# Alanlee0323/ISWM

Measured on AMD Instinct MI355X. Metric: training images/sec (513x513) DeepLabV3+-ResNet101, higher is better.
Workload: dtype f32; 1 GPU; deeplabv3plus_resnet101 output_stride=16, 513x513 synthetic tiles, 16 images/GPU (BASELINE.json configs[2]: global batch 128 over 8 GPUs), weighted CE [1,3], SGD-nesterov + cosine LR; fp32 tensors, conv products via six bf16 MFMAs on an exact 3-way operand split (bf16x6, fp32-level error); conv_math=bf16x6, global_batch=16, parallelism=dp1

## Files before the change

include/iswm_hip.h:

```cpp
#ifndef ISWM_HIP_H
#define ISWM_HIP_H

#include <stddef.h>
#include <stdint.h>

#ifdef __cplusplus
extern "C" {
#endif

typedef void* iswm_stream_t;

const char* iswm_last_error(void);
int iswm_version(void);

typedef struct {
    int N, H, W, Cin;
    int Ho, Wo, Cout;
    int KH, KW, stride, pad, dil;
    int ldx;
    int ldy;
} iswm_conv_desc;

int iswm_set_conv_math(int mode);
int iswm_get_conv_math(void);
// ... 25 lines not shown
int iswm_conv2d_dgrad_packed(const iswm_conv_desc* d, const float* dy, const void* wpk, float* dx, int accumulate,
                             iswm_stream_t stream);
int iswm_split_planes(const float* x, int64_t M, int C, int ldx, void* planes, int ldp, int64_t plane_stride,
                      iswm_stream_t stream);
int iswm_join_planes(const void* planes, int ldp, int64_t plane_stride, int64_t M, int C, float* x, int ldx,
                     iswm_stream_t stream);
int iswm_bn_apply_pl(const float* y, int64_t M, int C, int ldy, const float* scale, const float* shift, const float* mean,
                     const void* residual, int ldr, int64_t res_ps, int relu, void* out, int ldo, int64_t out_ps,
                     iswm_stream_t stream);
int iswm_bn_backward_pl(const float* dout, int ldd, const void* out, int ldo, int64_t out_ps, const float* y, int ldy,
                        int64_t M, int C, const float* mean, const float* invstd, const float* gamma,
                        const float* mask_scale, const float* mask_shift, int relu, int training, float* dgamma,
                        float* dbeta, void* dy, int lddy, int64_t dy_ps, float* dres, int lddres, void* workspace,
                        size_t workspace_bytes, iswm_stream_t stream);
int iswm_maxpool3x3s2_fwd_pl(const float* x, int N, int H, int W, int C, void* y, int64_t y_ps, uint8_t* idx, int Ho,
                             int Wo, iswm_stream_t stream);
int iswm_gap_fwd_pl(const void* x, int64_t x_ps, int N, int HW, int C, int ldx, float* y, iswm_stream_t stream);
int iswm_bcast_fwd_pl(const float* v, int N, int HW, int C, void* y, int ldy, int64_t y_ps, iswm_stream_t stream);
int iswm_bilinear_fwd_pl(const float* x, int N, int Hi, int Wi, int C, int ldx, void* y, int64_t y_ps, int Ho, int Wo,
                         int ldy, iswm_stream_t stream);
size_t iswm_conv2d_pl2_weight_bytes(const iswm_conv_desc* d, int kind);
int iswm_conv2d_pl2_pack_weights(const iswm_conv_desc* d, int kind, const float* w, void* packed, iswm_stream_t stream);
int iswm_conv2d_pl2_tile_rows(const iswm_conv_desc* d, int kind);
int iswm_conv2d_fwd_pl2(const iswm_conv_desc* d, const void* xp, int64_t plane_stride, const void* wpk,
                        const float* bias, float* y, float* stat_partials, iswm_stream_t stream);
int iswm_conv2d_dgrad_pl2(const iswm_conv_desc* d, const void* dyp, int64_t plane_stride, const void* wpk,
                          float* dx, int accumulate, iswm_stream_t stream);
int iswm_conv2d_dgrad_pl2_stat_tiles(const iswm_conv_desc* d);
int iswm_conv2d_dgrad_pl2_bn(const iswm_conv_desc* d, const void* dyp, int64_t plane_stride, const void* wpk, float* dx,
                             int accumulate, const float* y, int ldy, const float* mean, const float* invstd,
                             const float* mask_scale, const float* mask_shift, int relu, const void* mask_hi,
                             int ld_mask, double* partials, int tiles, iswm_stream_t stream);
int iswm_bn_backward_stats_pl(const float* dout, int ldd, const void* out, int ldo, int64_t out_ps, const float* y, int ldy,
                              int64_t M, int C, const float* mean, const float* invstd, const float* gamma,
                              const float* mask_scale, const float* mask_shift, int relu, int training, float* dgamma,
                              float* dbeta, void* dy, int lddy, int64_t dy_ps, float* dres, int lddres,
                              const double* partials, int tiles, void* workspace, size_t workspace_bytes,
                              iswm_stream_t stream);
size_t iswm_aspp_plan_bytes(const iswm_conv_desc* d, int nbranch, const int* ksize, const int* dil, int kind);
int iswm_aspp_plan(const iswm_conv_desc* d, int nbranch, const int* ksize, const int* dil, int kind, void* host_plan,
                   int grid_hint);
int iswm_aspp_fwd(const iswm_conv_desc* d, int nbranch, const int* ksize, const int* dil, const void* plan_dev, const void* xp,
                  int64_t x_ps, const void* const* wpk, float* const* y, float* const* stats, iswm_stream_t stream);
int iswm_aspp_bwd(const iswm_conv_desc* d, int nbranch, const int* ksize, const int* dil, const void* plan_dev, const void* dyp,
                  int64_t dy_ps, int ld_dy, const void* const* wpk, float* dx, int accumulate, const void* xp, int64_t x_ps,
                  float* const* dw, float* workspace, size_t workspace_bytes, iswm_stream_t stream);
// ... 198 lines not shown
```

iswm_amd/_lib.py:

```python
import ctypes
import os
from ctypes import POINTER, Structure, c_char_p, c_double, c_float, c_int, c_int64, c_size_t, c_uint64, c_void_p

HERE = os.path.dirname(os.path.abspath(__file__))
LIB_PATH = os.path.join(HERE, "libiswm_hip.so")


class ConvDesc(Structure):
    _fields_ = [(n, c_int) for n in ("N", "H", "W", "Cin", "Ho", "Wo", "Cout", "KH", "KW", "stride", "pad",
                                     "dil", "ldx", "ldy")]


class QConvDesc(Structure):
    _fields_ = [(n, c_int) for n in ("N", "H", "W", "Cin", "Ho", "Wo", "Cout", "KH", "KW", "stride", "pad",
                                     "dil", "ldx", "ldy", "ldr", "relu", "lo", "out_f32", "cstore")]


P = c_void_p
_SIGS = {
    "iswm_last_error": (c_char_p, []),
    "iswm_version": (c_int, []),
    "iswm_set_conv_math": (c_int, [c_int]),
    "iswm_get_conv_math": (c_int, []),
    "iswm_conv2d_kernel_name": (c_int, [POINTER(ConvDesc), c_int, c_char_p, c_int]),
# ... 4 lines not shown
    "iswm_transpose_weights": (c_int, [POINTER(ConvDesc), P, P, P]),
    "iswm_conv2d_dgrad_wants_wt": (c_int, [POINTER(ConvDesc)]),
    "iswm_conv2d_dgrad_wt": (c_int, [POINTER(ConvDesc), P, P, P, c_int, P]),
    "iswm_conv2d_packed_weight_bytes": (c_size_t, [POINTER(ConvDesc), c_int]),
    "iswm_conv2d_pack_weights": (c_int, [POINTER(ConvDesc), c_int, P, P, P]),
    "iswm_packed_weight_bytes": (c_size_t, [c_int, c_int, c_int, c_int]),
    "iswm_pack_job_blocks": (c_int, [c_int, c_int, c_int, c_int]),
    "iswm_pack_weights_batch": (c_int, [P, c_int, c_int, P]),
    "iswm_conv2d_fwd_packed_stat_layout": (c_int, [POINTER(ConvDesc), POINTER(c_int), POINTER(c_int)]),
    "iswm_conv2d_fwd_packed": (c_int, [POINTER(ConvDesc), P, P, P, P, P, P]),
    "iswm_conv2d_dgrad_packed": (c_int, [POINTER(ConvDesc), P, P, P, c_int, P]),
    "iswm_split_planes": (c_int, [P, c_int64, c_int, c_int, P, c_int, c_int64, P]),
    "iswm_join_planes": (c_int, [P, c_int, c_int64, c_int64, c_int, P, c_int, P]),
    "iswm_bn_apply_pl": (c_int, [P, c_int64, c_int, c_int, P, P, P, P, c_int, c_int64, c_int, P, c_int, c_int64, P]),
    "iswm_bn_backward_pl": (c_int, [P, c_int, P, c_int, c_int64, P, c_int, c_int64, c_int, P, P, P, P, P, c_int, c_int, P, P, P,
                                    c_int, c_int64, P, c_int, P, c_size_t, P]),
    "iswm_maxpool3x3s2_fwd_pl": (c_int, [P, c_int, c_int, c_int, c_int, P, c_int64, P, c_int, c_int, P]),
    "iswm_gap_fwd_pl": (c_int, [P, c_int64, c_int, c_int, c_int, c_int, P, P]),
    "iswm_bcast_fwd_pl": (c_int, [P, c_int, c_int, c_int, P, c_int, c_int64, P]),
    "iswm_bilinear_fwd_pl": (c_int, [P, c_int, c_int, c_int, c_int, c_int, P, c_int64, c_int, c_int, c_int, P]),
    "iswm_conv2d_pl2_weight_bytes": (c_size_t, [POINTER(ConvDesc), c_int]),
    "iswm_conv2d_pl2_pack_weights": (c_int, [POINTER(ConvDesc), c_int, P, P, P]),
    "iswm_conv2d_pl2_tile_rows": (c_int, [POINTER(ConvDesc), c_int]),
    "iswm_conv2d_fwd_pl2": (c_int, [POINTER(ConvDesc), P, c_int64, P, P, P, P, P]),
    "iswm_conv2d_dgrad_pl2": (c_int, [POINTER(ConvDesc), P, c_int64, P, P, c_int, P]),
    "iswm_conv2d_dgrad_pl2_stat_tiles": (c_int, [POINTER(ConvDesc)]),
    "iswm_conv2d_dgrad_pl2_bn": (c_int, [POINTER(ConvDesc), P, c_int64, P, P, c_int, P, c_int, P, P, P, P, c_int, P, c_int, P,
                                         c_int, P]),
    "iswm_bn_backward_stats_pl": (c_int, [P, c_int, P, c_int, c_int64, P, c_int, c_int64, c_int, P, P, P, P, P, c_int, c_int, P, P,
                                          P, c_int, c_int64, P, c_int, P, c_int, P, c_size_t, P]),
    "iswm_aspp_plan_bytes": (c_size_t, [POINTER(ConvDesc), c_int, POINTER(c_int), POINTER(c_int), c_int]),
    "iswm_aspp_plan": (c_int, [POINTER(ConvDesc), c_int, POINTER(c_int), POINTER(c_int), c_int, P, c_int]),
    "iswm_aspp_fwd": (c_int, [POINTER(ConvDesc), c_int, POINTER(c_int), POINTER(c_int), P, P, c_int64, POINTER(c_void_p),
                              POINTER(c_void_p), POINTER(c_void_p), P]),
    "iswm_aspp_bwd": (c_int, [POINTER(ConvDesc), c_int, POINTER(c_int), POINTER(c_int), P, P, c_int64, c_int, POINTER(c_void_p), P,
                              c_int, P, c_int64, POINTER(c_void_p), P, c_size_t, P]),
    "iswm_conv2d_wgrad_planes_ok": (c_int, [POINTER(ConvDesc)]),
    "iswm_conv2d_wgrad_planes_workspace": (c_size_t, [POINTER(ConvDesc)]),
    "iswm_conv2d_wgrad_planes": (c_int, [POINTER(ConvDesc), P, c_int64, P, c_int64, P, P, c_size_t, P]),
    "iswm_conv2d_wgrad_workspace": (c_size_t, [POINTER(ConvDesc)]),
    "iswm_dwconv2d_fwd": (c_int, [POINTER(ConvDesc), P, P, c_int, P, P, P]),
    "iswm_dwconv2d_dgrad": (c_int, [POINTER(ConvDesc), P, P, c_int, P, c_int, P]),
    "iswm_dwconv2d_wgrad_workspace": (c_size_t, [POINTER(ConvDesc)]),
    "iswm_dwconv2d_wgrad": (c_int, [POINTER(ConvDesc), P, P, c_int, P, P, c_size_t, P]),
    "iswm_dwconv3x3_stat_tile_rows": (c_int, [POINTER(ConvDesc)]),
    "iswm_dwconv3x3_stat_tiles": (c_int, [POINTER(ConvDesc)]),
# ... 114 lines not shown
```

iswm_amd/csrc/conv_api.hip:

```cpp
#include <stdlib.h>
#include <string.h>

#include <atomic>

#include "conv_common.h"

using namespace iswm;

static std::atomic<int> g_conv_math{-1};
static int conv_math() {
    int m = g_conv_math.load();
    if (m < 0) {
        const char* e = getenv("ISWM_CONV_MATH");
        const int env = (e && (!strcmp(e, "f32") || !strcmp(e, "0"))) ? 0
                        : (e && (!strcmp(e, "bf16") || !strcmp(e, "2"))) ? 2 : 1;
        int unset = -1;
        g_conv_math.compare_exchange_strong(unset, env);
        m = g_conv_math.load();
    }
    return m;
}
extern "C" int iswm_set_conv_math(int mode) {
    ISWM_REQUIRE(mode >= 0 && mode <= 2, "set_conv_math: mode must be 0 (f32), 1 (bf16x6) or 2 (bf16)");
    g_conv_math = mode;
// ... 200 lines not shown
    return route_name(plan_route(d, kind == 1 && dgrad_wants_wt(d, math) ? E_DGRAD_WT : entry[kind], math), buf, buflen);
}

extern "C" int iswm_conv2d_stat_tile_rows(const iswm_conv_desc* d) {
    return d ? plan_route(d, E_FWD, conv_math()).tile_rows : 0;
}

extern "C" int iswm_conv2d_stat_tiles(const iswm_conv_desc* d) {
    return d ? plan_route(d, E_FWD, conv_math()).tiles : 0;
}

extern "C" int iswm_conv2d_fwd_packed_stat_layout(const iswm_conv_desc* d, int* tiles, int* tile_rows) {
    ISWM_REQUIRE(d && tiles && tile_rows, "fwd_packed_stat_layout: null pointer");
    const ConvRoute r = plan_route(d, E_FWD_PACKED, conv_math());
    *tiles = r.tiles;
    *tile_rows = r.tile_rows;
    return 0;
}

extern "C" int iswm_conv2d_pl2_tile_rows(const iswm_conv_desc* d, int kind) {
    return d ? plan_route(d, kind ? E_DGRAD_PL2 : E_FWD_PL2, conv_math()).tile_rows : 0;
}

extern "C" int iswm_conv2d_dgrad_pl2_stat_tiles(const iswm_conv_desc* d) {
    return (d && d->Cin > 0) ? plan_route(d, E_DGRAD_PL2, conv_math()).stat_tiles : 0;
}

extern "C" size_t iswm_conv2d_wgrad_workspace(const iswm_conv_desc* d) {
    return d ? plan_wgrad(d, conv_math()).workspace : 0;
}

extern "C" int iswm_conv2d_fwd(const iswm_conv_desc* d, const float* x, const float* w, const float* bias,
                               float* y, float* stat_partials, iswm_stream_t stream) {
    if (int e = validate(d)) return e;
    ISWM_REQUIRE(x && w && y, "conv_fwd: null pointer");
    ISWM_REQUIRE(aligned16(x) && aligned16(w) && aligned16(y), "conv_fwd: pointers must be 16-byte aligned");
    ConvArgs a = base_args(d);
    a.x = x; a.w = w; a.bias = bias; a.y = y; a.stats = stat_partials;
    hipStream_t s = (hipStream_t)stream;
    const ConvRoute r = plan_route(d, E_FWD, conv_math());
    switch (r.family) {
    case F_STEM:
        ISWM_REQUIRE(launch_stem_fwd(a, s), "conv_fwd: the stem kernel does not cover this geometry");
        return check_launch("stem_fwd");
    case F_X6:
        ISWM_REQUIRE(launch_conv_fwd_x6(a, s, r.bm, r.bn), "conv_fwd: no bf16x6 kernel for tile %d x %d", r.bm, r.bn);
// ... 243 lines not shown
```

iswm_amd/csrc/conv_common.h:

```cpp
#pragma once
#include <stdlib.h>
#include "common.h"
#include "planes.h"

namespace iswm {

typedef float f32x16 __attribute__((ext_vector_type(16)));

struct BnFuse {
    const float* y;
    const float* mean;
    const float* invstd;
    const float* mscale;
    const float* mshift;
    double* part;
    int ldy, relu;
    const unsigned short* mask;
    int ldm;
};

struct ConvArgs {
    const float* x;
    const float* w;
    const float* bias;
// ... 96 lines not shown
    for (int i = 0; i < 8; ++i) {
        float x = 0.f;
        if (col < NC) x = DGRAD ? w[((size_t)(g0 + i) * T + tap) * Cin + col] : w[((size_t)col * T + tap) * Cin + g0 + i];
        v[i] = x;
    }
    uint4* o = packed + (size_t)f * (64 * NP) + lane;
    if constexpr (NP == 1) {
        const uint2 r0 = round_bf16x4(make_float4(v[0], v[1], v[2], v[3])), r1 = round_bf16x4(make_float4(v[4], v[5], v[6], v[7]));
        o[0] = make_uint4(r0.x, r0.y, r1.x, r1.y);
    } else {
        uint2 h0, m0, l0, h1, m1, l1;
        split3(make_float4(v[0], v[1], v[2], v[3]), h0, m0, l0);
        split3(make_float4(v[4], v[5], v[6], v[7]), h1, m1, l1);
        o[0] = make_uint4(h0.x, h0.y, h1.x, h1.y);
        o[64] = make_uint4(m0.x, m0.y, m1.x, m1.y);
        o[128] = make_uint4(l0.x, l0.y, l1.x, l1.y);
    }
}

int pack_job_blocks_pl2(int Cout, int T, int Cin, bool dgrad);
void conv_pl2_plan(int64_t M, int cols, int K, bool wide_ok, int* rbw, int* wide, int* wm);
bool launch_conv_pl2w(ConvArgs a, hipStream_t s, bool dgrad, int planes, int rbw);
bool launch_conv_pl2(ConvArgs a, hipStream_t s, bool dgrad, int planes, int rbw, int wm);
size_t packed_weight_bytes_pl2(int Cout, int T, int Cin, bool dgrad, int planes);
void launch_pack_weights_pl2(const float* w, void* packed, int Cout, int T, int Cin, bool dgrad, int planes, hipStream_t s);

struct PatchArgs {
    const float* x;
    const uint4* wpk;
    const float* bias;
    float* y;
    float* stats;
    int N, RH, RW;
    int GH, GW;
    int GC, NC;
    int KH, KW, dil;
    int orgh, orgw;
    int flip;
    int PH, PW, HH, HW;
    int TPY, TPX;
    int ldg, ldo;
    int MT, NT;
    int accumulate;
};
bool conv_patch_plan(int RH, int RW, int KH, int KW, int dil, int* PH, int* PW);
void launch_conv_x6_patch(PatchArgs a, bool dgrad, int planes, hipStream_t s);
// ... 28 lines not shown
```

iswm_amd/csrc/conv_mfma_pl2.hip:

```cpp
#include <stdlib.h>

#include "conv_pl2_stage.h"

namespace iswm {

constexpr int PL2_RBWMAX = 10;
constexpr double PL2W_EFF = 0.85;

template <int RBW, int WM, int NP, bool DGRAD>
__global__ __launch_bounds__(512, 2) void k_conv_pl2(const ConvArgs a) {
    const int GC = DGRAD ? a.Cout : a.Cin;
    const int NC = DGRAD ? a.Cin : a.Cout;
    constexpr int WN = 8 / WM, BN = 16 * WN;
    using S = Pl2Stage<16 * RBW * WM, NP>;
    constexpr int BM = S::BM, RG = S::RG, NRG = S::NRG, PLANE = S::PLANE, STAGE = S::STAGE;
    constexpr int XTRA = (DGRAD ? BM * 4 : 0) + (WM > 1 ? 4 * 128 * 4 : 0);
    __shared__ __attribute__((aligned(1024))) unsigned char smem[2 * STAGE + XTRA];
    int* rowpix = reinterpret_cast<int*>(smem + 2 * STAGE);
    float* red = reinterpret_cast<float*>(smem + 2 * STAGE + (DGRAD ? BM * 4 : 0));
    const unsigned lds_base = (unsigned)(uintptr_t)(lds_vptr)smem;

    const int t = threadIdx.x, lane = t & 63;
    const int wave = __builtin_amdgcn_readfirstlane(t >> 6);
    const int wm = wave / WN, wn = wave - wm * WN;
    const bool par = DGRAD && a.stride == 2 && a.psplit == 0;
    const int RH = DGRAD ? a.H : a.Ho, RW = DGRAD ? a.W : a.Wo;
    const int GH = DGRAD ? a.Ho : a.H, GW = DGRAD ? a.Wo : a.W;
    const int taps = a.KH * a.KW;
    const int nCC = GC >> 6;
    const int K32 = a.Ktot >> 5;
    const int ntiles = a.MT * a.NT;
    const unsigned char* xb = reinterpret_cast<const unsigned char*>(a.x);
    const int gs = pl2_dma_group(lane, wave);
    const unsigned char* zrow = reinterpret_cast<const unsigned char*>(g_zero_row_pl2) + gs * 16;

    int i_tile = xcd_remap(blockIdx.x, gridDim.x);
    int i_m0 = 0, i_n0 = 0;
    int ihb[NRG], iwb[NRG], pb[NRG];
    const uint4* wpk = nullptr;
    auto par_mt = [&](int sq) __attribute__((always_inline)) -> int {
        const int qn = a.MT >> 2, rem = a.MT & 3;
        int k = 0;
#pragma unroll
        for (int j = 0; j < 4; ++j) {
            k = (a.porder >> (2 * j)) & 3;
            const int sz = qn + (k < rem ? 1 : 0);
            if (sq < sz || j == 3) break;
            sq -= sz;
        }
        return k * qn + (k < rem ? k : rem) + sq;
    };
    auto load_tile = [&](int tile) __attribute__((always_inline)) {
        int mt = tile / a.NT;
        const int nt = tile - mt * a.NT;
        if (par) mt = par_mt(mt);
        i_m0 = mt * BM;
        i_n0 = nt * BN;
#pragma unroll
        for (int i = 0; i < NRG; ++i) {
            const int m = i_m0 + 8 * (wave + 8 * i) + (lane >> 3);
            if (wave + 8 * i < RG && m < a.M) {
                int n, rh, rw;
                x6_row_pixel(m, a.N, RH, RW, par, n, rh, rw);
                ihb[i] = DGRAD ? rh + a.pad : rh * a.stride - a.pad;
                iwb[i] = DGRAD ? rw + a.pad : rw * a.stride - a.pad;
                pb[i] = n * GH * GW;
            } else {
                ihb[i] = PL2_NO_ROW;
                iwb[i] = 0;
                pb[i] = 0;
            }
        }
        wpk = reinterpret_cast<const uint4*>(a.w) + (size_t)((i_n0 >> 4) + wn) * K32 * (64 * NP) + lane;
    };
    const unsigned char* aptr[NRG];
    int astep[NRG];
    long long pst[NRG];
    auto setup_tap = [&](int tap) __attribute__((always_inline)) -> bool {
        const int kh = tap / a.KW, kw = tap - kh * a.KW;
        const int dh = kh * a.dil, dw = kw * a.dil;
        int any = 0;
#pragma unroll
        for (int i = 0; i < NRG; ++i) {
            int gh, gw;
            bool ok;
            if (DGRAD) {
                int th = ihb[i] - dh, tw = iwb[i] - dw;
                gh = th;
                gw = tw;
                ok = th >= 0 && tw >= 0;
                if (a.stride != 1) {
                    gh = th / a.stride;
                    gw = tw / a.stride;
                    ok = ok && (gh * a.stride == th) && (gw * a.stride == tw);
                }
                ok = ok && gh < GH && gw < GW;
            } else {
                gh = ihb[i] + dh;
                gw = iwb[i] + dw;
                ok = (unsigned)gh < (unsigned)GH && (unsigned)gw < (unsigned)GW;
            }
// ... 53 lines not shown
            asrc[i] = more ? aptr[i] : zrow;
            apl[i] = more ? pst[i] : 0;
        }
        auto slot = [&](int sidx) __attribute__((always_inline)) {
            if (sidx < NB_SLOTS) {
                bn.v[sidx / NP][sidx % NP] = wn_[sidx * 64];
            } else if (sidx < NSLOTS) {
                const int i = (sidx - NB_SLOTS) / NP, pp = (sidx - NB_SLOTS) % NP;
                if (8 * i + 8 <= RG || wave + 8 * i < RG)
                    glds16b(asrc[i] + pp * apl[i], lds_base + (st ^ 1) * STAGE + pp * PLANE + (wave + 8 * i) * 1024);
                if (pp == NP - 1) aptr[i] += astep[i];
            }
        };
        Pl2AFrag<NP> f[3];
        pl2_aload<S, RBW>(f[0], smem, st, fbase, 0);
        pl2_aload<S, RBW>(f[1], smem, st, fbase, 1);
#pragma unroll
        for (int idx = 0; idx < 2 * RBW; ++idx) {
            if (idx + 2 < 2 * RBW) pl2_aload<S, RBW>(f[(idx + 2) % 3], smem, st, fbase, idx + 2);
            __builtin_amdgcn_sched_barrier(0);
            pl2_mul(acc[idx % RBW], b.v[idx / RBW], f[idx % 3]);
#pragma unroll
            for (int q = 0; q < PER; ++q) slot(idx * PER + q);
            __builtin_amdgcn_sched_barrier(0);
        }
    };

    const int lq = lane >> 4, lp = lane & 15;
    auto epilogue = [&](int tile, int m0, int n0, bool zero) __attribute__((always_inline)) {
        int mt = tile / a.NT;
        if (par) mt = par_mt(mt);
        const int col = n0 + 16 * wn + 4 * lq;
        const bool cok = col < NC;
        const bool bnf = DGRAD && a.bnf.part != nullptr;
        const bool mk = bnf && a.bnf.relu == 3;
        if (DGRAD && a.accumulate && zero && !bnf) return;
        float4 bv = make_float4(0.f, 0.f, 0.f, 0.f);
        if (!DGRAD && a.bias != nullptr && cok) bv = *reinterpret_cast<const float4*>(a.bias + col);
        if (DGRAD && par) {
            __syncthreads();
            if (t < BM) {
                const int m = m0 + t;
                int n = 0, rh = 0, rw = 0;
                if (m < a.M) x6_row_pixel(m, a.N, RH, RW, true, n, rh, rw);
                rowpix[DGRAD ? t : 0] = (n * RH + rh) * RW + rw;
            }
// ... 172 lines not shown
            for (int i = 0; i < RBW; ++i) acc[i] = f32x4{0.f, 0.f, 0.f, 0.f};
        }
    };

    int c_tile = i_tile, c_m0, c_n0;
    load_tile(i_tile);
    c_m0 = i_m0;
    c_n0 = i_n0;
    auto next_tile = [&]() __attribute__((always_inline)) -> bool {
        i_tile += gridDim.x;
        if (i_tile >= ntiles) return false;
        load_tile(i_tile);
        tap = -1;
        cc = nCC - 1;
        return true;
    };
    auto next_tile_stage = [&]() __attribute__((always_inline)) -> bool {
        for (;;) {
            if (!next_tile()) return false;
            if (next_in_tile()) return true;
            epilogue(i_tile, i_m0, i_n0, true);
        }
    };
    {
        BFrag bc, bn;
        bool have = next_in_tile();
        if (!have) {
            epilogue(i_tile, i_m0, i_n0, true);
            have = next_tile_stage();
            c_tile = i_tile; c_m0 = i_m0; c_n0 = i_n0;
        }
        if (have) {
            bload(bc, tap * (GC >> 5) + 2 * cc);
            issueA(0);
        }
        int st = 0;
        while (have) {
            __builtin_amdgcn_s_waitcnt(0x0F70);
            __builtin_amdgcn_s_barrier();
            asm volatile("" ::: "memory");
            bool more = next_in_tile();
            const bool last = !more;
            if (last) more = next_tile_stage();
            compute(st, bc, more, bn, more ? tap * (GC >> 5) + 2 * cc : 0);
            if (last) {
                epilogue(c_tile, c_m0, c_n0, false);
                c_tile = i_tile; c_m0 = i_m0; c_n0 = i_n0;
// ... 20 lines not shown
            best = rbw;
        }
    }
    return best;
}

void conv_pl2_plan(int64_t M, int cols, int K, bool wide_ok, int* rbw_out, int* wide_out, int* wm_out) {
    *wm_out = cols <= 64 ? 2 : 1;
    *rbw_out = conv_pl2_pick_rbw(M, cols, *wm_out);
    *wide_out = 0;
    if (!wide_ok || cols < 256 || K < 256) return;
    const int64_t NT = (cols + 127) / 128, NTW = (cols + 255) / 256;
    const int64_t MT0 = (M + *rbw_out * 16 - 1) / (*rbw_out * 16);
    double best = (double)((MT0 * NT + 255) / 256) * (*rbw_out * 16 + 24.0);
    for (int rbw = 8; rbw <= PL2_RBWMAX; ++rbw) {
        const int64_t MT = (M + rbw * 16 - 1) / (rbw * 16);
        const double c = (double)((MT * NTW + 255) / 256) * (rbw * 16 + 24.0) * 2.0 * PL2W_EFF;
        if (c < best - 1e-9) {
            best = c;
            *rbw_out = rbw;
            *wide_out = 1;
        }
    }
}

bool launch_conv_pl2(ConvArgs a, hipStream_t s, bool dgrad, int planes, int rbw, int wm) {
    a.psplit = 0;
    {
        int wgt[4], ord[4] = {0, 1, 2, 3};
        for (int k = 0; k < 4; ++k) {
            int ch = 0, cw = 0;
            for (int kh = 0; kh < a.KH; ++kh) ch += (((k >> 1) + a.pad - kh * a.dil) & 1) == 0;
            for (int kw = 0; kw < a.KW; ++kw) cw += (((k & 1) + a.pad - kw * a.dil) & 1) == 0;
            wgt[k] = ch * cw;
        }
        for (int i = 0; i < 4; ++i)
            for (int j = i + 1; j < 4; ++j)
                if (wgt[ord[j]] > wgt[ord[i]]) { const int t = ord[i]; ord[i] = ord[j]; ord[j] = t; }
        a.porder = ord[0] | (ord[1] << 2) | (ord[2] << 4) | (ord[3] << 6);
    }
    const int nc = dgrad ? a.Cin : a.Cout;
    const bool narrow = wm == 2;
    a.MT = (a.M + rbw * 16 - 1) / (rbw * 16);
    a.NT = narrow ? 1 : (nc + 127) / 128;
    const int tiles = a.MT * a.NT, ncu = device_cus();
    dim3 grid(tiles < ncu ? tiles : ncu), blk(512);
    if (planes != 1 && planes != 3) return false;
#define PL2_LAUNCH(R, W)                                                                       \
    do {                                                                                       \
        if (planes == 1) {                                                                     \
            if (dgrad) hipLaunchKernelGGL((k_conv_pl2<R, W, 1, true>), grid, blk, 0, s, a);     \
            else hipLaunchKernelGGL((k_conv_pl2<R, W, 1, false>), grid, blk, 0, s, a);          \
        } else {                                                                               \
            if (dgrad) hipLaunchKernelGGL((k_conv_pl2<R, W, 3, true>), grid, blk, 0, s, a);     \
            else hipLaunchKernelGGL((k_conv_pl2<R, W, 3, false>), grid, blk, 0, s, a);          \
        }                                                                                      \
    } while (0)
    if (narrow) {
        if (rbw == 8) PL2_LAUNCH(4, 2);
        else if (rbw == 10) PL2_LAUNCH(5, 2);
        else return false;
    } else {
        if (rbw == 8) PL2_LAUNCH(8, 1);
        else if (rbw == 9) PL2_LAUNCH(9, 1);
        else if (rbw == 10) PL2_LAUNCH(10, 1);
        else return false;
    }
#undef PL2_LAUNCH
    return true;
}

template <bool DGRAD, int NP>
__global__ __launch_bounds__(256) void k_pack_weights_pl2(const float* __restrict__ w, uint4* __restrict__ packed, int Cout,
                                                          int T, int Cin, int K32, int total) {
    const int idx = blockIdx.x * 256 + threadIdx.x;
    if (idx >= total) return;
    pack_weights_pl2_body<DGRAD, NP>(w, packed, Cout, T, Cin, K32, idx);
}

int pack_job_blocks_pl2(int Cout, int T, int Cin, bool dgrad) {
    const int NC = dgrad ? Cin : Cout, GC = dgrad ? Cout : Cin;
// ... 27 lines not shown
```

iswm_amd/csrc/conv_mfma_pl2w.hip:

```cpp
#include <stdlib.h>

#include "conv_pl2_stage.h"

namespace iswm {

template <int RBW, int NP, bool DGRAD>
__global__ __launch_bounds__(512, 2) void k_conv_pl2w(const ConvArgs a) {
    const int GC = DGRAD ? a.Cout : a.Cin;
    const int NC = DGRAD ? a.Cin : a.Cout;
    using S = Pl2Stage<16 * RBW, NP>;
    constexpr int BM = S::BM, RG = S::RG, NRG = S::NRG, PLANE = S::PLANE, STAGE = S::STAGE;
    __shared__ __attribute__((aligned(1024))) unsigned char smem[2 * STAGE];
    const unsigned lds_base = (unsigned)(uintptr_t)(lds_vptr)smem;

    const int t = threadIdx.x, lane = t & 63;
    const int wave = __builtin_amdgcn_readfirstlane(t >> 6);
    const int RH = DGRAD ? a.H : a.Ho, RW = DGRAD ? a.W : a.Wo;
    const int GH = DGRAD ? a.Ho : a.H, GW = DGRAD ? a.Wo : a.W;
    const int taps = a.KH * a.KW;
    const int nCC = GC >> 6;
    const int K32 = a.Ktot >> 5;
    const int ntiles = a.MT * a.NT;
    const int cbs = ((NC + 127) >> 7) << 3;
    const unsigned char* xb = reinterpret_cast<const unsigned char*>(a.x);
    const int gs = pl2_dma_group(lane, wave);
    const unsigned char* zrow = reinterpret_cast<const unsigned char*>(g_zero_row_pl2) + gs * 16;

    int i_tile = xcd_remap(blockIdx.x, gridDim.x);
    int i_m0 = 0, i_n0 = 0;
    int ihb[NRG], iwb[NRG], pb[NRG];
    const uint4* wpk[2] = {nullptr, nullptr};
    auto load_tile = [&](int tile) __attribute__((always_inline)) {
        const int mt = tile / a.NT;
        const int nt = tile - mt * a.NT;
        i_m0 = mt * BM;
        i_n0 = nt * 256;
#pragma unroll
        for (int i = 0; i < NRG; ++i) {
            const int m = i_m0 + 8 * (wave + 8 * i) + (lane >> 3);
            if (wave + 8 * i < RG && m < a.M) {
                int n, rh, rw;
                x6_row_pixel(m, a.N, RH, RW, false, n, rh, rw);
                ihb[i] = DGRAD ? rh + a.pad : rh * a.stride - a.pad;
                iwb[i] = DGRAD ? rw + a.pad : rw * a.stride - a.pad;
                pb[i] = n * GH * GW;
            } else {
                ihb[i] = PL2_NO_ROW;
                iwb[i] = 0;
                pb[i] = 0;
            }
        }
#pragma unroll
        for (int cb = 0; cb < 2; ++cb) {
            const int cbi = min((i_n0 >> 4) + 2 * wave + cb, cbs - 1);
            wpk[cb] = reinterpret_cast<const uint4*>(a.w) + (size_t)cbi * K32 * (64 * NP) + lane;
        }
    };
    const unsigned char* aptr[NRG];
    int astep[NRG];
    long long pst[NRG];
    auto setup_tap = [&](int tap) __attribute__((always_inline)) -> bool {
        const int kh = tap / a.KW, kw = tap - kh * a.KW;
        const int dh = kh * a.dil, dw = kw * a.dil;
        int any = 0;
#pragma unroll
        for (int i = 0; i < NRG; ++i) {
            int gh, gw;
            bool ok;
            if (DGRAD) {
                gh = ihb[i] - dh;
                gw = iwb[i] - dw;
                ok = gh >= 0 && gw >= 0 && gh < GH && gw < GW;
            } else {
                gh = ihb[i] + dh;
                gw = iwb[i] + dw;
                ok = (unsigned)gh < (unsigned)GH && (unsigned)gw < (unsigned)GW;
            }
            aptr[i] = ok ? xb + ((size_t)(pb[i] + gh * GW + gw) * a.ldx) * 2 + gs * 16 : zrow;
            astep[i] = ok ? 128 : 0;
            pst[i] = ok ? a.xps : 0;
            any |= ok;
        }
        if (a.pad < 4) return true;
        return __syncthreads_or(any) != 0;
// ... 75 lines not shown
                const int cb = s / NP, pl = s - cb * NP;
                if (half == 0) B[cb][1][pl] = (cb ? wc1 : wc0)[(NP + pl) * 64];
                else B[cb][0][pl] = (cb ? wn1 : wn0)[pl * 64];
            } else {
                const int j = s - NB;
                if (half == 0) { if (j < NA0) dma(j); }
                else { if (j < NA1) dma(NA0 + j); }
            }
        };
        Pl2AFrag<NP> f[3];
        aload(f[0], 0);
        aload(f[1], 1);
#pragma unroll
        for (int idx = 0; idx < 2 * RBW; ++idx) {
            if (idx + 2 < 2 * RBW) aload(f[(idx + 2) % 3], idx + 2);
            __builtin_amdgcn_sched_barrier(0);
            mul(f[idx % 3], idx);
            const int half = idx / RBW, rb = idx - half * RBW;
            slot(half, 2 * rb);
            slot(half, 2 * rb + 1);
            __builtin_amdgcn_sched_barrier(0);
        }
        static_assert(2 * RBW >= NB + NA1, "load slots do not fit the row blocks of a k half");
    };

    const int lq = lane >> 4, lp = lane & 15;
    auto epilogue = [&](int tile, int m0, int n0, bool zero) __attribute__((always_inline)) {
        const int mt = tile / a.NT;
        const bool bnf = DGRAD && a.bnf.part != nullptr;
        const bool mk = bnf && a.bnf.relu == 3;
        if (DGRAD && a.accumulate && zero && !bnf) return;
#pragma unroll
        for (int cb = 0; cb < 2; ++cb) {
            const int col = n0 + 32 * wave + 16 * cb + 4 * lq;
            const bool cok = col < NC;
            float4 bv = make_float4(0.f, 0.f, 0.f, 0.f);
            if (!DGRAD && a.bias != nullptr && cok) bv = *reinterpret_cast<const float4*>(a.bias + col);
            float4 f_mu = make_float4(0.f, 0.f, 0.f, 0.f), f_is = f_mu, f_sc = f_mu, f_sh = f_mu;
            float fs[4] = {0.f, 0.f, 0.f, 0.f}, fq[4] = {0.f, 0.f, 0.f, 0.f};
            if (bnf && cok) {
                f_mu = *reinterpret_cast<const float4*>(a.bnf.mean + col);
                f_is = *reinterpret_cast<const float4*>(a.bnf.invstd + col);
                if (a.bnf.relu == 2) {
                    f_sc = *reinterpret_cast<const float4*>(a.bnf.mscale + col);
                    f_sh = *reinterpret_cast<const float4*>(a.bnf.mshift + col);
                }
// ... 136 lines not shown
                for (int i = 0; i < RBW; ++i) acc[cb][i] = f32x4{0.f, 0.f, 0.f, 0.f};
        }
    };

    int c_tile = i_tile, c_m0, c_n0;
    load_tile(i_tile);
    c_m0 = i_m0;
    c_n0 = i_n0;
    auto next_tile = [&]() __attribute__((always_inline)) -> bool {
        i_tile += gridDim.x;
        if (i_tile >= ntiles) return false;
        load_tile(i_tile);
        tap = -1;
        cc = nCC - 1;
        return true;
    };
    auto next_tile_stage = [&]() __attribute__((always_inline)) -> bool {
        for (;;) {
            if (!next_tile()) return false;
            if (next_in_tile()) return true;
            epilogue(i_tile, i_m0, i_n0, true);
        }
    };
    {
        bool have = next_in_tile();
        if (!have) {
            epilogue(i_tile, i_m0, i_n0, true);
            have = next_tile_stage();
            c_tile = i_tile; c_m0 = i_m0; c_n0 = i_n0;
        }
        if (have) {
            k32_c = tap * (GC >> 5) + 2 * cc;
            wpk_c[0] = wpk[0];
            wpk_c[1] = wpk[1];
            bload_half(wpk, k32_c, 0);
            issueA(0);
        }
        int st = 0;
        while (have) {
            __builtin_amdgcn_s_waitcnt(0x0F70);
            __builtin_amdgcn_s_barrier();
            asm volatile("" ::: "memory");
            bool more = next_in_tile();
            const bool last = !more;
            if (last) more = next_tile_stage();
            const int k32n = more ? tap * (GC >> 5) + 2 * cc : 0;
            compute(st, more, k32n);
// ... 4 lines not shown
            st ^= 1;
            k32_c = k32n;
            wpk_c[0] = wpk[0];
            wpk_c[1] = wpk[1];
            have = more;
        }
    }
    __builtin_amdgcn_s_waitcnt(0x0F70);
}

bool launch_conv_pl2w(ConvArgs a, hipStream_t s, bool dgrad, int planes, int rbw) {
    if (planes != 3 || (dgrad && a.stride != 1)) return false;
    const int nc = dgrad ? a.Cin : a.Cout;
    a.MT = (a.M + rbw * 16 - 1) / (rbw * 16);
    a.NT = (nc + 255) / 256;
    a.psplit = 1;
    const int tiles = a.MT * a.NT, ncu = device_cus();
    dim3 grid(tiles < ncu ? tiles : ncu), blk(512);
#define PL2W_LAUNCH(R)                                                                     \
    do {                                                                                   \
        if (dgrad) hipLaunchKernelGGL((k_conv_pl2w<R, 3, true>), grid, blk, 0, s, a);       \
        else hipLaunchKernelGGL((k_conv_pl2w<R, 3, false>), grid, blk, 0, s, a);            \
    } while (0)
    if (rbw == 8) PL2W_LAUNCH(8);
    else if (rbw == 9) PL2W_LAUNCH(9);
    else if (rbw == 10) PL2W_LAUNCH(10);
    else return false;
#undef PL2W_LAUNCH
    return true;
}

}
```

Before: 277.5 images/sec.

## Add band path for 3x3 stride-1 convs reusing one staged row band across kw taps

For 3x3 stride-1 convolutions with pad equal to dilation (dil 1 to 3), both pl2 kernels gain a BAND variant. It stages a contiguous band of BM plus 8 pixel rows into LDS once per kh tap and reads it three times at shifted LDS offsets for the three kw taps. Width-boundary pixels are zeroed with per-row masks. This cuts the number of global-to-LDS stages per K step from nine taps to three, reducing global load traffic and barrier count. In exchange it uses a slightly larger stage buffer, adds mask ALU work on the fragments, and brings a new scheduling path that carries correctness risk around row wraparound.

```diff
diff --git a/include/iswm_hip.h b/include/iswm_hip.h
--- a/include/iswm_hip.h
+++ b/include/iswm_hip.h
@@ -71,6 +71,7 @@
 size_t iswm_conv2d_pl2_weight_bytes(const iswm_conv_desc* d, int kind);
 int iswm_conv2d_pl2_pack_weights(const iswm_conv_desc* d, int kind, const float* w, void* packed, iswm_stream_t stream);
 int iswm_conv2d_pl2_tile_rows(const iswm_conv_desc* d, int kind);
+int iswm_conv2d_band_taps(const iswm_conv_desc* d, int entry_point);
 int iswm_conv2d_fwd_pl2(const iswm_conv_desc* d, const void* xp, int64_t plane_stride, const void* wpk,
                         const float* bias, float* y, float* stat_partials, iswm_stream_t stream);
 int iswm_conv2d_dgrad_pl2(const iswm_conv_desc* d, const void* dyp, int64_t plane_stride, const void* wpk,
diff --git a/iswm_amd/_lib.py b/iswm_amd/_lib.py
--- a/iswm_amd/_lib.py
+++ b/iswm_amd/_lib.py
@@ -50,6 +50,7 @@
     "iswm_conv2d_pl2_weight_bytes": (c_size_t, [POINTER(ConvDesc), c_int]),
     "iswm_conv2d_pl2_pack_weights": (c_int, [POINTER(ConvDesc), c_int, P, P, P]),
     "iswm_conv2d_pl2_tile_rows": (c_int, [POINTER(ConvDesc), c_int]),
+    "iswm_conv2d_band_taps": (c_int, [POINTER(ConvDesc), c_int]),
     "iswm_conv2d_fwd_pl2": (c_int, [POINTER(ConvDesc), P, c_int64, P, P, P, P, P]),
     "iswm_conv2d_dgrad_pl2": (c_int, [POINTER(ConvDesc), P, c_int64, P, P, c_int, P]),
     "iswm_conv2d_dgrad_pl2_stat_tiles": (c_int, [POINTER(ConvDesc)]),
diff --git a/iswm_amd/csrc/conv_api.hip b/iswm_amd/csrc/conv_api.hip
--- a/iswm_amd/csrc/conv_api.hip
+++ b/iswm_amd/csrc/conv_api.hip
@@ -246,6 +246,17 @@
     return d ? plan_route(d, kind ? E_DGRAD_PL2 : E_FWD_PL2, conv_math()).tile_rows : 0;
 }
 
+extern "C" int iswm_conv2d_band_taps(const iswm_conv_desc* d, int entry_point) {
+    const int math = conv_math();
+    if (!d || math < 1 || (entry_point != 0 && entry_point != 1)) return 0;
+    if (d->KH <= 0 || d->KW <= 0 || d->stride <= 0 || d->dil <= 0 || d->pad < 0 || d->N <= 0 || d->H <= 0 || d->W <= 0) return 0;
+    if ((entry_point ? d->Cout : d->Cin) <= 0 || (entry_point ? d->Cout : d->Cin) % 64 != 0) return 0;
+    if ((entry_point ? d->Cin : d->Cout) <= 0) return 0;
+    const ConvRoute r = plan_route(d, entry_point ? E_DGRAD_PL2 : E_FWD_PL2, math);
+    if (r.family != F_PL2 && r.family != F_PL2W) return 0;
+    return conv_pl2_band(base_args(d, entry_point == 1), r.planes, r.wm, r.family == F_PL2W) ? 1 : 0;
+}
+
 extern "C" int iswm_conv2d_dgrad_pl2_stat_tiles(const iswm_conv_desc* d) {
     return (d && d->Cin > 0) ? plan_route(d, E_DGRAD_PL2, conv_math()).stat_tiles : 0;
 }
diff --git a/iswm_amd/csrc/conv_common.h b/iswm_amd/csrc/conv_common.h
--- a/iswm_amd/csrc/conv_common.h
+++ b/iswm_amd/csrc/conv_common.h
@@ -142,6 +142,7 @@
 void conv_pl2_plan(int64_t M, int cols, int K, bool wide_ok, int* rbw, int* wide, int* wm);
 bool launch_conv_pl2w(ConvArgs a, hipStream_t s, bool dgrad, int planes, int rbw);
 bool launch_conv_pl2(ConvArgs a, hipStream_t s, bool dgrad, int planes, int rbw, int wm);
+bool conv_pl2_band(const ConvArgs& a, int planes, int wm, bool wide);
 size_t packed_weight_bytes_pl2(int Cout, int T, int Cin, bool dgrad, int planes);
 void launch_pack_weights_pl2(const float* w, void* packed, int Cout, int T, int Cin, bool dgrad, int planes, hipStream_t s);
 
diff --git a/iswm_amd/csrc/conv_mfma_pl2.hip b/iswm_amd/csrc/conv_mfma_pl2.hip
--- a/iswm_amd/csrc/conv_mfma_pl2.hip
+++ b/iswm_amd/csrc/conv_mfma_pl2.hip
@@ -7,14 +7,17 @@
 constexpr int PL2_RBWMAX = 10;
 constexpr double PL2W_EFF = 0.85;
 
-template <int RBW, int WM, int NP, bool DGRAD>
+template <int RBW, int WM, int NP, bool DGRAD, bool BAND = false>
 __global__ __launch_bounds__(512, 2) void k_conv_pl2(const ConvArgs a) {
     const int GC = DGRAD ? a.Cout : a.Cin;
     const int NC = DGRAD ? a.Cin : a.Cout;
     constexpr int WN = 8 / WM, BN = 16 * WN;
-    using S = Pl2Stage<16 * RBW * WM, NP>;
-    constexpr int BM = S::BM, RG = S::RG, NRG = S::NRG, PLANE = S::PLANE, STAGE = S::STAGE;
+    constexpr int BM = 16 * RBW * WM;
+    using S = Pl2Stage<BM + (BAND ? 8 : 0), NP>;
+    constexpr int RG = S::RG, NRG = S::NRG, PLANE = S::PLANE, STAGE = S::STAGE;
     constexpr int XTRA = (DGRAD ? BM * 4 : 0) + (WM > 1 ? 4 * 128 * 4 : 0);
+    static_assert(2 * STAGE + XTRA <= 160 * 1024, "k_conv_pl2: stage buffers exceed the LDS of a CU");
+    static_assert(!BAND || NRG == 3, "k_conv_pl2<BAND>: one row group of the band per kw sub-stage");
     __shared__ __attribute__((aligned(1024))) unsigned char smem[2 * STAGE + XTRA];
     int* rowpix = reinterpret_cast<int*>(smem + 2 * STAGE);
     float* red = reinterpret_cast<float*>(smem + 2 * STAGE + (DGRAD ? BM * 4 : 0));
@@ -23,10 +26,10 @@
     const int t = threadIdx.x, lane = t & 63;
     const int wave = __builtin_amdgcn_readfirstlane(t >> 6);
     const int wm = wave / WN, wn = wave - wm * WN;
-    const bool par = DGRAD && a.stride == 2 && a.psplit == 0;
+    const bool par = !BAND && DGRAD && a.stride == 2 && a.psplit == 0;
     const int RH = DGRAD ? a.H : a.Ho, RW = DGRAD ? a.W : a.Wo;
     const int GH = DGRAD ? a.Ho : a.H, GW = DGRAD ? a.Wo : a.W;
-    const int taps = a.KH * a.KW;
+    const int taps = BAND ? 3 : a.KH * a.KW;
     const int nCC = GC >> 6;
     const int K32 = a.Ktot >> 5;
     const int ntiles = a.MT * a.NT;
@@ -58,6 +61,14 @@
         i_n0 = nt * BN;
 #pragma unroll
         for (int i = 0; i < NRG; ++i) {
+            if constexpr (BAND) {
+                const int m = i_m0 - a.dil + 8 * (wave + 8 * i) + (lane >> 3);
+                const bool in = wave + 8 * i < RG && m >= 0 && m < a.M;
+                ihb[i] = in ? (m / RW) % RH : PL2_NO_ROW;
+                iwb[i] = 0;
+                pb[i] = in ? m : 0;
+                continue;
+            }
             const int m = i_m0 + 8 * (wave + 8 * i) + (lane >> 3);
             if (wave + 8 * i < RG && m < a.M) {
                 int n, rh, rw;
@@ -77,6 +88,17 @@
     int astep[NRG];
     long long pst[NRG];
     auto setup_tap = [&](int tap) __attribute__((always_inline)) -> bool {
+        if constexpr (BAND) {
+            const int dh = (DGRAD ? 1 - tap : tap - 1) * a.dil;
+#pragma unroll
+            for (int i = 0; i < NRG; ++i) {
+                const bool ok = (unsigned)(ihb[i] + dh) < (unsigned)GH;
+                aptr[i] = ok ? xb + ((size_t)(pb[i] + dh * GW) * a.ldx) * 2 + gs * 16 : zrow;
+                astep[i] = ok ? 128 : 0;
+                pst[i] = ok ? a.xps : 0;
+            }
+            return true;
+        }
         const int kh = tap / a.KW, kw = tap - kh * a.KW;
         const int dh = kh * a.dil, dw = kw * a.dil;
         int any = 0;
@@ -176,6 +198,76 @@
             pl2_mul(acc[idx % RBW], b.v[idx / RBW], f[idx % 3]);
 #pragma unroll
             for (int q = 0; q < PER; ++q) slot(idx * PER + q);
+            __builtin_amdgcn_sched_barrier(0);
+        }
+    };
+
+    unsigned mk_l = 0, mk_r = 0;
+    int fb3[3] = {0, 0, 0};
+    if constexpr (BAND) {
+#pragma unroll
+        for (int kw = 0; kw < 3; ++kw) {
+            const int r = wm * (RBW * 16) + (lane & 15) + (DGRAD ? 2 - kw : kw) * a.dil;
+            fb3[kw] = r * 128 + (((lane >> 4) ^ ((r >> 1) & 7)) * 16);
+        }
+    }
+    auto band_masks = [&](int m0) __attribute__((always_inline)) {
+        int ow = (m0 + wm * (RBW * 16) + (lane & 15)) % RW;
+        const int step = 16 % RW;
+        mk_l = mk_r = 0;
+#pragma unroll
+        for (int rb = 0; rb < RBW; ++rb) {
+            mk_l |= (ow >= a.dil ? 1u : 0u) << rb;
+            mk_r |= (ow + a.dil < RW ? 1u : 0u) << rb;
+            ow += step;
+            ow = ow >= RW ? ow - RW : ow;
+        }
+    };
+    auto compute_band = [&](int st, BFrag& b0, BFrag& b1, bool more, const uint4* wcur, int k32c, int k32n) __attribute__((always_inline)) {
+        constexpr int NB_SLOTS = 2 * NP, NSLOTS = NB_SLOTS + NP, NI = 2 * RBW;
+        constexpr int PER = (NSLOTS + NI - 1) / NI;
+        const int G = GC >> 5;
+        const uint4* wsrc[3] = {wcur + (size_t)(k32c + G) * (64 * NP), wcur + (size_t)(k32c + 2 * G) * (64 * NP),
+                                wpk + (size_t)k32n * (64 * NP)};
+        const unsigned char* asrc[NRG];
+        long long apl[NRG];
+#pragma unroll
+        for (int i = 0; i < NRG; ++i) {
+            asrc[i] = more ? aptr[i] : zrow;
+            apl[i] = more ? pst[i] : 0;
+        }
+        Pl2AFrag<NP> f[3];
+        pl2_aload<S, RBW>(f[0], smem, st, fb3[0], 0);
+        pl2_aload<S, RBW>(f[1], smem, st, fb3[0], 1);
+#pragma unroll
+        for (int g = 0; g < 3 * NI; ++g) {
+            const int kw = g / NI, idx = g - kw * NI;
+            if (g + 2 < 3 * NI) pl2_aload<S, RBW>(f[(g + 2) % 3], smem, st, fb3[(g + 2) / NI], (g + 2) % NI);
+            __builtin_amdgcn_sched_barrier(0);
+            Pl2AFrag<NP> fm = f[g % 3];
+            if (kw != 1) {
+                const unsigned mb = ((kw == 0) != DGRAD) ? mk_l : mk_r;
+                const unsigned mw = (unsigned)((int)(mb << (31 - idx % RBW)) >> 31);
+#pragma unroll
+                for (int pl = 0; pl < NP; ++pl) {
+                    fm.v[pl].x &= mw; fm.v[pl].y &= mw; fm.v[pl].z &= mw; fm.v[pl].w &= mw;
+                }
+            }
+            const BFrag& b = kw == 1 ? b1 : b0;
+            BFrag& bl = kw == 1 ? b0 : b1;
+            pl2_mul(acc[idx % RBW], b.v[idx / RBW], fm);
+#pragma unroll
+            for (int q = 0; q < PER; ++q) {
+                const int sidx = idx * PER + q;
+                if (sidx < NB_SLOTS) {
+                    bl.v[sidx / NP][sidx % NP] = wsrc[kw][sidx * 64];
+                } else if (sidx < NSLOTS) {
+                    const int pp = sidx - NB_SLOTS;
+                    if (8 * kw + 8 <= RG || wave + 8 * kw < RG)
+                        glds16b(asrc[kw] + pp * apl[kw], lds_base + (st ^ 1) * STAGE + pp * PLANE + (wave + 8 * kw) * 1024);
+                    if (pp == NP - 1) aptr[kw] += astep[kw];
+                }
+            }
             __builtin_amdgcn_sched_barrier(0);
         }
     };
@@ -394,7 +486,36 @@
             epilogue(i_tile, i_m0, i_n0, true);
         }
     };
-    {
+    if constexpr (BAND) {
+        BFrag bc, bn;
+        next_in_tile();
+        int kc = 3 * tap * (GC >> 5) + 2 * cc;
+        bload(bc, kc);
+        issueA(0);
+        band_masks(c_m0);
+        int st = 0;
+        bool have = true;
+        while (have) {
+            __builtin_amdgcn_s_waitcnt(0x0F70);
+            __builtin_amdgcn_s_barrier();
+            asm volatile("" ::: "memory");
+            const uint4* wcur = wpk;
+            bool more = next_in_tile();
+            const bool last = !more;
+            if (last) more = next_tile_stage();
+            const int kn = more ? 3 * tap * (GC >> 5) + 2 * cc : 0;
+            compute_band(st, bc, bn, more, wcur, kc, kn);
+            if (last) {
+                epilogue(c_tile, c_m0, c_n0, false);
+                c_tile = i_tile; c_m0 = i_m0; c_n0 = i_n0;
+                band_masks(c_m0);
+            }
+            st ^= 1;
+            bc = bn;
+            kc = kn;
+            have = more;
+        }
+    } else {
         BFrag bc, bn;
         bool have = next_in_tile();
         if (!have) {
@@ -461,6 +582,10 @@
             *wide_out = 1;
         }
     }
+}
+
+bool conv_pl2_band(const ConvArgs& a, int planes, int wm, bool wide) {
+    return planes == 3 && (wide || wm == 2) && a.KH == 3 && a.KW == 3 && a.stride == 1 && a.pad == a.dil && a.dil >= 1 && a.dil <= 3;
 }
 
 bool launch_conv_pl2(ConvArgs a, hipStream_t s, bool dgrad, int planes, int rbw, int wm) {
@@ -495,7 +620,17 @@
             else hipLaunchKernelGGL((k_conv_pl2<R, W, 3, false>), grid, blk, 0, s, a);          \
         }                                                                                      \
     } while (0)
-    if (narrow) {
+    if (conv_pl2_band(a, planes, wm, false)) {
+#define PL2_LAUNCH_BAND(R, W)                                                                  \
+    do {                                                                                       \
+        if (dgrad) hipLaunchKernelGGL((k_conv_pl2<R, W, 3, true, true>), grid, blk, 0, s, a);   \
+        else hipLaunchKernelGGL((k_conv_pl2<R, W, 3, false, true>), grid, blk, 0, s, a);        \
+    } while (0)
+        if (rbw == 8) PL2_LAUNCH_BAND(4, 2);
+        else if (rbw == 10) PL2_LAUNCH_BAND(5, 2);
+        else return false;
+#undef PL2_LAUNCH_BAND
+    } else if (narrow) {
         if (rbw == 8) PL2_LAUNCH(4, 2);
         else if (rbw == 10) PL2_LAUNCH(5, 2);
         else return false;
diff --git a/iswm_amd/csrc/conv_mfma_pl2w.hip b/iswm_amd/csrc/conv_mfma_pl2w.hip
--- a/iswm_amd/csrc/conv_mfma_pl2w.hip
+++ b/iswm_amd/csrc/conv_mfma_pl2w.hip
@@ -1,15 +1,20 @@
 #include <stdlib.h>
 
+#include <type_traits>
+
 #include "conv_pl2_stage.h"
 
 namespace iswm {
 
-template <int RBW, int NP, bool DGRAD>
+template <int RBW, int NP, bool DGRAD, bool BAND = false>
 __global__ __launch_bounds__(512, 2) void k_conv_pl2w(const ConvArgs a) {
     const int GC = DGRAD ? a.Cout : a.Cin;
     const int NC = DGRAD ? a.Cin : a.Cout;
-    using S = Pl2Stage<16 * RBW, NP>;
-    constexpr int BM = S::BM, RG = S::RG, NRG = S::NRG, PLANE = S::PLANE, STAGE = S::STAGE;
+    constexpr int BM = 16 * RBW;
+    using S = Pl2Stage<BM + (BAND ? 8 : 0), NP>;
+    constexpr int RG = S::RG, NRG = S::NRG, PLANE = S::PLANE, STAGE = S::STAGE;
+    static_assert(2 * STAGE <= 160 * 1024, "k_conv_pl2w: stage buffers exceed the LDS of a CU");
+    static_assert(!BAND || NRG == 3, "k_conv_pl2w<BAND>: one row group of the band per kw sub-stage");
     __shared__ __attribute__((aligned(1024))) unsigned char smem[2 * STAGE];
     const unsigned lds_base = (unsigned)(uintptr_t)(lds_vptr)smem;
 
@@ -17,7 +22,7 @@
     const int wave = __builtin_amdgcn_readfirstlane(t >> 6);
     const int RH = DGRAD ? a.H : a.Ho, RW = DGRAD ? a.W : a.Wo;
     const int GH = DGRAD ? a.Ho : a.H, GW = DGRAD ? a.Wo : a.W;
-    const int taps = a.KH * a.KW;
+    const int taps = BAND ? 3 : a.KH * a.KW;
     const int nCC = GC >> 6;
     const int K32 = a.Ktot >> 5;
     const int ntiles = a.MT * a.NT;
@@ -37,6 +42,14 @@
         i_n0 = nt * 256;
 #pragma unroll
         for (int i = 0; i < NRG; ++i) {
+            if constexpr (BAND) {
+                const int m = i_m0 - a.dil + 8 * (wave + 8 * i) + (lane >> 3);
+                const bool in = wave + 8 * i < RG && m >= 0 && m < a.M;
+                ihb[i] = in ? (m / RW) % RH : PL2_NO_ROW;
+                iwb[i] = 0;
+                pb[i] = in ? m : 0;
+                continue;
+            }
             const int m = i_m0 + 8 * (wave + 8 * i) + (lane >> 3);
             if (wave + 8 * i < RG && m < a.M) {
                 int n, rh, rw;
@@ -60,6 +73,17 @@
     int astep[NRG];
     long long pst[NRG];
     auto setup_tap = [&](int tap) __attribute__((always_inline)) -> bool {
+        if constexpr (BAND) {
+            const int dh = (DGRAD ? 1 - tap : tap - 1) * a.dil;
+#pragma unroll
+            for (int i = 0; i < NRG; ++i) {
+                const bool ok = (unsigned)(ihb[i] + dh) < (unsigned)GH;
+                aptr[i] = ok ? xb + ((size_t)(pb[i] + dh * GW) * a.ldx) * 2 + gs * 16 : zrow;
+                astep[i] = ok ? 128 : 0;
+                pst[i] = ok ? a.xps : 0;
+            }
+            return true;
+        }
         const int kh = tap / a.KW, kw = tap - kh * a.KW;
         const int dh = kh * a.dil, dw = kw * a.dil;
         int any = 0;
@@ -181,6 +205,85 @@
             __builtin_amdgcn_sched_barrier(0);
         }
         static_assert(2 * RBW >= NB + NA1, "load slots do not fit the row blocks of a k half");
+    };
+
+    unsigned mk_l = 0, mk_r = 0;
+    int fb3[3] = {0, 0, 0};
+    if constexpr (BAND) {
+#pragma unroll
+        for (int kw = 0; kw < 3; ++kw) {
+            const int r = (lane & 15) + (DGRAD ? 2 - kw : kw) * a.dil;
+            fb3[kw] = r * 128 + (((lane >> 4) ^ ((r >> 1) & 7)) * 16);
+        }
+    }
+    auto band_masks = [&](int m0) __attribute__((always_inline)) {
+        int ow = (m0 + (lane & 15)) % RW;
+        const int step = 16 % RW;
+        mk_l = mk_r = 0;
+#pragma unroll
+        for (int rb = 0; rb < RBW; ++rb) {
+            mk_l |= (ow >= a.dil ? 1u : 0u) << rb;
+            mk_r |= (ow + a.dil < RW ? 1u : 0u) << rb;
+            ow += step;
+            ow = ow >= RW ? ow - RW : ow;
+        }
+    };
+    auto compute_band = [&](int st, bool more, int k32n) __attribute__((always_inline)) {
+        constexpr int NB = 2 * NP, NA0 = NP / 2, NA1 = NP - NA0, NI = 2 * RBW;
+        static_assert(2 * RBW >= NB + NA1, "load slots do not fit the row blocks of a k half");
+        const int G = GC >> 5;
+        const unsigned char* asrc[NRG];
+        long long apl[NRG];
+#pragma unroll
+        for (int i = 0; i < NRG; ++i) {
+            asrc[i] = more ? aptr[i] : zrow;
+            apl[i] = more ? pst[i] : 0;
+        }
+        auto slot = [&](int kw, int half, int s) __attribute__((always_inline)) {
+            if (s < NB) {
+                const int cb = s / NP, pl = s - cb * NP;
+                if (half == 0) B[cb][1][pl] = (wpk_c[cb] + (size_t)(k32_c + kw * G) * (64 * NP))[(NP + pl) * 64];
+                else if (kw < 2) B[cb][0][pl] = (wpk_c[cb] + (size_t)(k32_c + (kw + 1) * G) * (64 * NP))[pl * 64];
+                else B[cb][0][pl] = (wpk[cb] + (size_t)k32n * (64 * NP))[pl * 64];
+            } else {
+                const int j = s - NB, pp = half == 0 ? j : NA0 + j;
+                if (j < (half == 0 ? NA0 : NA1)) {
+                    if (8 * kw + 8 <= RG || wave + 8 * kw < RG)
+                        glds16b(asrc[kw] + pp * apl[kw], lds_base + (st ^ 1) * STAGE + pp * PLANE + (wave + 8 * kw) * 1024);
+                    if (pp == NP - 1) aptr[kw] += astep[kw];
+                }
+            }
+        };
+        Pl2AFrag<NP> f[3];
+        pl2_aload<S, RBW>(f[0], smem, st, fb3[0], 0);
+        pl2_aload<S, RBW>(f[1], smem, st, fb3[0], 1);
+        auto sub = [&](auto KW) __attribute__((always_inline)) {
+        constexpr int kw = decltype(KW)::value;
+#pragma unroll
+        for (int idx = 0; idx < NI; ++idx) {
+            const int g = kw * NI + idx;
+            const int half = idx / RBW, rb = idx - half * RBW;
+            if (g + 2 < 3 * NI) pl2_aload<S, RBW>(f[(g + 2) % 3], smem, st, fb3[(g + 2) / NI], (g + 2) % NI);
+            __builtin_amdgcn_sched_barrier(0);
+            Pl2AFrag<NP> fm = f[g % 3];
+            if (kw != 1) {
+                const unsigned mb = ((kw == 0) != DGRAD) ? mk_l : mk_r;
+                const unsigned mw = (unsigned)((int)(mb << (31 - rb)) >> 31);
+#pragma unroll
+                for (int pl = 0; pl < NP; ++pl) {
+                    fm.v[pl].x &= mw; fm.v[pl].y &= mw; fm.v[pl].z &= mw; fm.v[pl].w &= mw;
+                }
+            }
+#pragma unroll
+            for (int cb = 0; cb < 2; ++cb) pl2_mul(acc[cb][rb], B[cb][half], fm);
+            slot(kw, half, 2 * rb);
+            slot(kw, half, 2 * rb + 1);
+            __builtin_amdgcn_sched_barrier(0);
+        }
+        };
+        sub(std::integral_constant<int, 0>{});
+        sub(std::integral_constant<int, 1>{});
+        sub(std::integral_constant<int, 2>{});
     };
 
     const int lq = lane >> 4, lp = lane & 15;
@@ -363,7 +466,37 @@
             epilogue(i_tile, i_m0, i_n0, true);
         }
     };
-    {
+    if constexpr (BAND) {
+        next_in_tile();
+        k32_c = 3 * tap * (GC >> 5) + 2 * cc;
+        wpk_c[0] = wpk[0];
+        wpk_c[1] = wpk[1];
+        bload_half(wpk, k32_c, 0);
+        issueA(0);
+        band_masks(c_m0);
+        int st = 0;
+        bool have = true;
+        while (have) {
+            __builtin_amdgcn_s_waitcnt(0x0F70);
+            __builtin_amdgcn_s_barrier();
+            asm volatile("" ::: "memory");
+            bool more = next_in_tile();
+            const bool last = !more;
+            if (last) more = next_tile_stage();
+            const int k32n = more ? 3 * tap * (GC >> 5) + 2 * cc : 0;
+            compute_band(st, more, k32n);
+            if (last) {
+                epilogue(c_tile, c_m0, c_n0, false);
+                c_tile = i_tile; c_m0 = i_m0; c_n0 = i_n0;
+                band_masks(c_m0);
+            }
+            st ^= 1;
+            k32_c = k32n;
+            wpk_c[0] = wpk[0];
+            wpk_c[1] = wpk[1];
+            have = more;
+        }
+    } else {
         bool have = next_in_tile();
         if (!have) {
             epilogue(i_tile, i_m0, i_n0, true);
@@ -414,7 +547,18 @@
         if (dgrad) hipLaunchKernelGGL((k_conv_pl2w<R, 3, true>), grid, blk, 0, s, a);       \
         else hipLaunchKernelGGL((k_conv_pl2w<R, 3, false>), grid, blk, 0, s, a);            \
     } while (0)
-    if (rbw == 8) PL2W_LAUNCH(8);
+    if (conv_pl2_band(a, planes, 1, true)) {
+#define PL2W_LAUNCH_BAND(R)                                                                \
+    do {                                                                                   \
+        if (dgrad) hipLaunchKernelGGL((k_conv_pl2w<R, 3, true, true>), grid, blk, 0, s, a); \
+        else hipLaunchKernelGGL((k_conv_pl2w<R, 3, false, true>), grid, blk, 0, s, a);      \
+    } while (0)
+        if (rbw == 8) PL2W_LAUNCH_BAND(8);
+        else if (rbw == 9) PL2W_LAUNCH_BAND(9);
+        else if (rbw == 10) PL2W_LAUNCH_BAND(10);
+        else return false;
+#undef PL2W_LAUNCH_BAND
+    } else if (rbw == 8) PL2W_LAUNCH(8);
     else if (rbw == 9) PL2W_LAUNCH(9);
     else if (rbw == 10) PL2W_LAUNCH(10);
     else return false;
```

Result: no change. 276.9 images/sec (-0.2%).
